# cjpatton/janus

Measured on AMD Instinct MI355X. Metric: helper reports/sec (prep_init+aggregate), Prio3SumVec len=1000 @1/2/4/8 GPU, higher is better.
Workload: dtype u32 (Field128 mod-p integer arithmetic, Keccak-p[1600,12]); 1 GPU; Prio3SumVec bits=8 length=1000 chunk_length=88: helper prep_init + prep_shares_to_prep + prep_next + aggregate; reports_per_gpu=1250000, parallelism=report-sharded x1 (RCCL all-gather + device mod-p combine)

## Files before the change

### janus_amd/csrc/jx_engine.cpp

```cpp
#include <hip/hip_runtime.h>

#include <cstdio>
#include <cstdlib>
#include <cstring>
#include <map>
#include <mutex>
#include <set>
#include <string>
#include <unordered_map>
#include <unordered_set>
#include <vector>

#include "jx_engine_internal.h"
#include "jx_field.h"
#include "jx_fused_plan.h"
#include "jx_sha_aes.h"
#include "jx_upload.h"

using namespace jx;
using namespace jxi;

static thread_local std::string t_err;

namespace jxi {
// ... 175 lines not shown
  c.P = next_pow2(1 + c.calls);
  if (mp && c.P > (1u << 30)) {
    why = "too many gadget calls for Field64";
    return JX_E_UNSUPPORTED;
  }
  c.logP = ilog2(c.P);
  c.gpoly_len = 2 * (c.P - 1) + 1;
  c.proof_len = arity + c.gpoly_len;
  c.ver_len = arity + 2;
  if (fp) {
    c.proof1_off = c.proof_len;
    c.proof_len += c.chunk1 + c.gpoly1_len;
    c.ver_len += c.chunk1 + 1;
  }
  const uint32_t fb = (c.algo == ALGO_COUNT || mp) ? 8 : 16;
  c.fb = fb;
  const bool jr = c.jr_len > 0;
  const uint32_t S = c.seed;
  c.ps_bytes = jr ? 2 * S : 0;
  c.his_bytes = jr ? 3 * S : 2 * S;
  c.lps_bytes = c.np * c.ver_len * fb + (jr ? S : 0);
  c.lis_bytes = (c.meas_len + c.np * c.proof_len) * fb + (jr ? S : 0);
  if (mp) {
    c.nco = MCOEF_K + 2 * c.calls;
    c.ncoef = 0;
    host_hmac_pads(vk, c.vk_ist, c.vk_ost);
    const uint8_t zero[32] = {0};
    host_hmac_pads(zero, c.zero_ist, c.zero_ost);
  } else if (c.algo == ALGO_COUNT)
    c.ncoef = 0;
  else if (c.algo == ALGO_SUM)
    c.ncoef = COEF_K + c.calls;
  else
    c.ncoef = COEF_K + 2 * c.calls;
  if (c.algo == ALGO_SUMVEC || c.algo == ALGO_HISTOGRAM || fp) {
    c.c_rpow = c.ncoef;
    c.ncoef += c.chunk;
    c.c_tpow = c.ncoef;
    c.ncoef += c.ngroups;
  }
  if (fp) {
    c.coef1 = c.ncoef;
    c.ncoef += G1_K + c.calls1;
  }
  for (int i = 0; i < 4; i++)
    c.vk[i] = (uint32_t)vk[4 * i] | ((uint32_t)vk[4 * i + 1] << 8) | ((uint32_t)vk[4 * i + 2] << 16) |
              ((uint32_t)vk[4 * i + 3] << 24);
  c.c_omega = 0;
  c.c_S = c.P;
  c.c_misc = c.P + c.gpoly_len;
  c.c_omega1 = c.c_misc + NMISC;
  c.c_S1 = c.c_omega1 + c.P1;
  return JX_OK;
}

static uint4 h_u4_64(uint64_t v) {
  uint4 r;
  r.x = lo32(v);
  r.y = hi32(v);
  r.z = r.w = 0;
  return r;
}

static void root_tables(f128 gen, uint32_t P, uint32_t logP, uint32_t calls, uint32_t glen, uint4* omega, uint4* S) {
  f128 w = gen;
  for (int i = 0; i < 66 - (int)logP; i++) w = mont128(w, w);
  f128 wk = make128(R1_128_LO, R1_128_HI);
// ... 2079 lines not shown
```

### janus_amd/csrc/jx_field.h

```cpp
#pragma once
#include <stdint.h>

#if defined(__HIPCC__) || defined(__HIP__)
#include <hip/hip_runtime.h>
#define JX_HD __host__ __device__ __forceinline__
#else
#define JX_HD static inline
#endif

namespace jx {


struct f128 {
  uint64_t lo, hi;
};

#if defined(__HIP_DEVICE_COMPILE__)
JX_HD uint32_t xor3(uint32_t a, uint32_t b, uint32_t c) { return __builtin_amdgcn_bitop3_b32(a, b, c, 0x96); }
JX_HD uint32_t maj3(uint32_t a, uint32_t b, uint32_t c) { return __builtin_amdgcn_bitop3_b32(a, b, c, 0xE8); }
#else
JX_HD uint32_t xor3(uint32_t a, uint32_t b, uint32_t c) { return a ^ b ^ c; }
JX_HD uint32_t maj3(uint32_t a, uint32_t b, uint32_t c) { return (a & b) ^ (a & c) ^ (b & c); }
#endif
JX_HD uint32_t lo32(uint64_t v) { return (uint32_t)v; }
// ... 271 lines not shown
  uint32_t c = 0;
  uint64_t a1 = addc64(w1, w2 * 28u, c);
  uint32_t b1 = b;
  a1 = subb64(a1, 0, b1);
  const uint64_t k = (uint64_t)(c - b1);
  uint32_t b2 = 0;
  a0 = subb64(a0, k, b2);
  a1 = a1 + 28u * k - b2;
  f128 v = make128(a0, a1);
  uint32_t br = 0;
  const uint64_t lo = subb64(v.lo, P128_LO, br);
  const uint64_t hi = subb64(v.hi, P128_HI, br);
  return ge_p128(v) ? make128(lo, hi) : v;
}
JX_HD void acc_add128(acc192& a, f128 v) { acc_add(a, v.lo, v.hi, 0); }
JX_HD f128 acc_reduce(const acc192& a) { return reduce192(a.w0, a.w1, a.w2); }


struct limbs26 {
  uint32_t l[5];
};
JX_HD limbs26 to_limbs26(f128 a) {
  const uint32_t M = (1u << 26) - 1;
  const uint32_t w0 = lo32(a.lo), w1 = hi32(a.lo), w2 = lo32(a.hi), w3 = hi32(a.hi);
  limbs26 r;
  r.l[0] = w0 & M;
  r.l[1] = (uint32_t)(((((uint64_t)w1) << 32) | w0) >> 26) & M;
  r.l[2] = (uint32_t)(((((uint64_t)w2) << 32) | w1) >> 20) & M;
  r.l[3] = (uint32_t)(((((uint64_t)w3) << 32) | w2) >> 14) & M;
  r.l[4] = w3 >> 8;
  return r;
}

struct wacc26 {
  uint64_t col[9];
};
JX_HD void wacc_zero(wacc26& a) {
#pragma unroll
  for (int s = 0; s < 9; s++) a.col[s] = 0;
}
JX_HD void wacc_mac(wacc26& a, const limbs26& x, const limbs26& c) {
#pragma unroll
  for (int i = 0; i < 5; i++)
#pragma unroll
    for (int j = 0; j < 5; j++) {
      a.col[i + j] += (uint64_t)x.l[i] * c.l[j];
#ifdef __HIP_DEVICE_COMPILE__
      asm("" : "+v"(a.col[i + j]));
#endif
    }
}
JX_HD void wacc_normalize(wacc26& a) {
  const uint64_t M = (1ull << 26) - 1;
#pragma unroll
  for (int s = 0; s < 8; s++) {
    a.col[s + 1] += a.col[s] >> 26;
    a.col[s] &= M;
  }
}
JX_HD f128 wacc_reduce(wacc26 a) {
  wacc_normalize(a);
  uint64_t o[5] = {0, 0, 0, 0, 0};
  int oi = 0, nb = 0;
  uint64_t buf_lo = 0, buf_hi = 0;
#pragma unroll
  for (int s = 0; s < 9; s++) {
// ... 165 lines not shown
```

### janus_amd/csrc/jx_flp.hip

```cpp
#include "jx_field.h"
#include "jx_kernels.h"

namespace jx {


__device__ __forceinline__ f128 ld_lead(const Bufs& b, const Cfg& c, uint64_t r, uint32_t idx, bool& dfail) {
  uint4 v = *reinterpret_cast<const uint4*>(b.lps + (uint64_t)c.lps_bytes * r + 16u * idx);
  f128 x = u4_to_f(v);
  dfail |= ge_p128(x);
  return x;
}

template <bool LEADER>
__global__ __launch_bounds__(256) void flp_sum_kernel(Cfg c, Bufs b) {
  const uint32_t lane = threadIdx.x & 63;
  const uint64_t blk = (uint64_t)blockIdx.x * 4 + (threadIdx.x >> 6);
  const uint64_t nblk = (b.n + 63) / 64;
  if (blk >= nblk) return;
  const uint64_t r0 = blk * 64 + lane;
  const uint64_t r = r0 < b.n ? r0 : b.n - 1;
  const uint32_t NC = c.ncoef, C = c.calls;
  const uint4* omega = b.consts + c.c_omega;
  f128 LR = ld_il(b.coef, blk, NC, COEF_L, lane), c0R = ld_il(b.coef, blk, NC, COEF_C0, lane);
  f128 tR = ld_il(b.coef, blk, NC, COEF_T, lane), rR = ld_il(b.coef, blk, NC, COEF_R, lane);
  acc192 ao;
  acc_zero(ao);
  const MeasView mv = meas_view(c, b, blk, lane);
  for (uint32_t k = 1; k <= C; k++) {
    f128 x = u4_to_f(mv[k - 1]);
    uint64_t lo, hi;
    uint32_t top;
    mont128_lazy(x, ld_il(b.coef, blk, NC, COEF_K + k - 1, lane), lo, hi, top);
// ... 44 lines not shown
    }
    return;
  }
  bool dfail = false;
  f128 lv = ld_lead(b, c, r, 0, dfail), lw = ld_lead(b, c, r, 1, dfail), lg = ld_lead(b, c, r, 2, dfail);
  const uint32_t flags = b.flags[r];
  uint32_t verdict = 0;
  if (flags & FLAG_INIT_FAIL)
    verdict = 1;
  else if (dfail)
    verdict = 2;
  else {
    f128 V0 = add128(v, lv), V1 = add128(W0, lw), VG = add128(G, lg);
    f128 lhs = sub128(mont128(V1, V1), mont128(V1, make128(1, 0)));
    if (!is_zero128(V0) || !eq128(lhs, mont128(VG, make128(1, 0))))
      verdict = 3;
    else if (flags & FLAG_NEXT_FAIL)
      verdict = 4;
  }
  if (r0 < b.n) b.verdicts[r0] = (uint8_t)verdict;
}

template <int PPW, bool HIST, bool LEADER>
__device__ __forceinline__ void psum_group_finish(const Cfg& c, const Bufs& b, uint64_t blk, uint32_t g, uint32_t lane,
                                                  const f128* E, const f128* O, f128 sxr);
template <int PPW, bool HIST, bool LEADER>
__device__ __forceinline__ void psum_part_finish(const Cfg& c, const Bufs& b, uint64_t blk, uint32_t g, uint32_t lane,
                                                 uint32_t kf, wacc26* ae, wacc26* ao, acc192& sx) {
  const uint32_t NG = c.ngroups;
  const uint64_t r0 = blk * 64 + lane;
  const uint64_t r = r0 < b.n ? r0 : b.n - 1;
  const uint32_t NC = c.ncoef, C = c.calls, chunk = c.chunk, M = c.meas_len, A = 2 * chunk;
  const uint32_t j0 = g * PPW;
  const uint4* coefb = b.coef + il_idx(blk, NC, 0, lane);
  const MeasView measb = meas_view(c, b, blk, lane);
#pragma unroll 1
  for (uint32_t k = kf + 1; k <= C; k++) {
    const limbs26 ck = to_limbs26(u4_to_f(coefb[(COEF_K + 2 * (k - 1)) * IL]));
    const limbs26 dk = to_limbs26(u4_to_f(coefb[(COEF_K + 2 * (k - 1) + 1) * IL]));
    const uint32_t nb = (k - 1) * chunk + j0;
#pragma unroll
    for (int i = 0; i < PPW; i++) {
      if (j0 + i < chunk && nb + i < M) {
        const f128 x = u4_to_f(measb[nb + i]);
        const limbs26 xl = to_limbs26(x);
        wacc_mac(ae[i], xl, dk);
        wacc_mac(ao[i], xl, ck);
        if (HIST) acc_add128(sx, x);
      }
    }
    if (((k - kf) & 511u) == 0) {
#pragma unroll
      for (int i = 0; i < PPW; i++) {
        wacc_normalize(ae[i]);
        wacc_normalize(ao[i]);
      }
    }
  }
  f128 E[PPW], O[PPW];
#pragma unroll
  for (int i = 0; i < PPW; i++) {
    E[i] = wacc_reduce(ae[i]);
    O[i] = wacc_reduce(ao[i]);
  }
  psum_group_finish<PPW, HIST, LEADER>(c, b, blk, g, lane, E, O, HIST ? acc_reduce(sx) : make128(0, 0));
}

template <int PPW, bool HIST, bool LEADER>
__device__ __forceinline__ void psum_group_finish(const Cfg& c, const Bufs& b, uint64_t blk, uint32_t g, uint32_t lane,
                                                  const f128* E, const f128* O, f128 sxr) {
  const uint32_t NG = c.ngroups;
  const uint64_t r0 = blk * 64 + lane;
// ... 40 lines not shown
      gpart = add128(mont128(gpart, tR), gm);
    }
    gpart = mont128(gpart, u4_to_f(coefb[(c.c_tpow + g) * IL]));
  }
  uint4* pp = b.part + ((blk * c.ngt + g) * 4) * IL + lane;
  pp[0] = f_to_u4(prod);
  pp[IL] = f_to_u4(vpart);
  pp[2 * IL] = f_to_u4(gpart);
  if (HIST) pp[3 * IL] = f_to_u4(sxr);
  if (dfail && r0 < b.n) atomicOr(&b.flags[r0], FLAG_DFAIL);
}

template <int PPW, bool HIST, bool LEADER, int PF = 1>
__global__ __launch_bounds__(64, 4) void flp_psum_part_kernel(Cfg c, Bufs b) {
  const uint32_t NG = c.ngroups;
  const uint32_t bid = blockIdx.x;
  const uint32_t xcd = bid & 7u, q = bid >> 3;
  const uint32_t g = q % NG;
  const uint64_t blk = (uint64_t)(q / NG) * 8 + xcd;
  const uint64_t nblk = (b.n + 63) / 64;
  if (blk >= nblk) return;
  const uint32_t lane = threadIdx.x;
  const uint32_t NC = c.ncoef, C = c.calls, chunk = c.chunk, M = c.meas_len;
  const uint32_t j0 = g * PPW;

  wacc26 ae[PPW], ao[PPW];
  acc192 sx;
#pragma unroll
  for (int i = 0; i < PPW; i++) {
    wacc_zero(ae[i]);
    wacc_zero(ao[i]);
  }
  acc_zero(sx);
  const uint4* coefb = b.coef + il_idx(blk, NC, 0, lane);
  const MeasView measb = meas_view(c, b, blk, lane);
  uint32_t kf = 0;
  if (j0 + PPW <= chunk && M >= j0 + PPW) kf = min(C, (M - j0 - PPW) / chunk + 1);
  for (uint32_t k0 = 1; k0 <= kf; k0 += 512) {
    const uint32_t k1 = min(kf, k0 + 511);
    uint4 cr[PF], dr[PF], xr[PF][PPW];
#pragma unroll
    for (int u = 0; u < PF; u++) {
      const uint32_t k = k0 + u;
      if (k <= k1) {
        cr[u] = coefb[(COEF_K + 2 * (k - 1)) * IL];
        dr[u] = coefb[(COEF_K + 2 * (k - 1) + 1) * IL];
#pragma unroll
        for (int i = 0; i < PPW; i++) xr[u][i] = measb[(uint64_t)((k - 1) * chunk + j0 + i)];
      }
    }
#pragma unroll 1
    for (uint32_t kb = k0; kb <= k1; kb += PF) {
#pragma unroll
      for (int u = 0; u < PF; u++) {
        const uint32_t k = kb + u;
        if (k <= k1) {
          const limbs26 ck = to_limbs26(u4_to_f(cr[u]));
          const limbs26 dk = to_limbs26(u4_to_f(dr[u]));
          f128 x[PPW];
#pragma unroll
          for (int i = 0; i < PPW; i++) x[i] = u4_to_f(xr[u][i]);
          const uint32_t kn = k + PF;
          if (kn <= k1) {
            cr[u] = coefb[(COEF_K + 2 * (kn - 1)) * IL];
            dr[u] = coefb[(COEF_K + 2 * (kn - 1) + 1) * IL];
#pragma unroll
            for (int i = 0; i < PPW; i++) xr[u][i] = measb[(uint64_t)((kn - 1) * chunk + j0 + i)];
          }
#pragma unroll
          for (int i = 0; i < PPW; i++) {
            const limbs26 xl = to_limbs26(x[i]);
            wacc_mac(ae[i], xl, dk);
            wacc_mac(ao[i], xl, ck);
            if (HIST) acc_add128(sx, x[i]);
          }
        }
      }
    }
#pragma unroll
    for (int i = 0; i < PPW; i++) {
      wacc_normalize(ae[i]);
      wacc_normalize(ao[i]);
    }
  }
  psum_part_finish<PPW, HIST, LEADER>(c, b, blk, g, lane, kf, ae, ao, sx);
}

template <int N>
__device__ __forceinline__ void wait_vmcnt() {
  static_assert(N >= 0 && N < 64, "vmcnt is 6 bits");
  __builtin_amdgcn_s_waitcnt(0x3f70 | (N & 15) | ((N >> 4) << 14));
}
__device__ __forceinline__ void glds16(const uint4* src, uint4* lds_row) {
  __builtin_amdgcn_global_load_lds((const void*)src, (void*)lds_row, 16, 0, 0);
}

constexpr uint32_t K3W = 4;
__device__ __forceinline__ uint32_t lds_addr(const void* p) {
  return (uint32_t)(size_t)(const __attribute__((address_space(3))) uint8_t*)p;
}
__device__ __forceinline__ void lds_read4(uint32_t a0, uint32_t a1, uint32_t a2, uint32_t a3, uint4& v0, uint4& v1,
                                          uint4& v2, uint4& v3) {
  asm volatile(
      "ds_read_b128 %0, %4\n\t"
      "ds_read_b128 %1, %5\n\t"
      "ds_read_b128 %2, %6\n\t"
      "ds_read_b128 %3, %7\n\t"
      "s_waitcnt lgkmcnt(0)"
      : "=&v"(v0), "=&v"(v1), "=&v"(v2), "=&v"(v3)
      : "v"(a0), "v"(a1), "v"(a2), "v"(a3)
      : "memory");
}
template <int PPW, bool HIST, bool LEADER, int D, int W = K3W, bool RING_ONLY = false>
__global__ __launch_bounds__(64 * W, 4) void flp_psum_part_glds_kernel(Cfg c, Bufs b) {
  static_assert(PPW == 2, "lds_read4 reads c, d and two measurement rows");
  constexpr int ROWS = 2 + W * PPW;
  __shared__ uint4 ring[D][ROWS][64];
  const uint32_t NG = c.ngroups, NW = (NG + W - 1) / W;
  const uint32_t bid = blockIdx.x, xcd = bid & 7u, q = bid >> 3;
  const uint32_t wg = q % NW;
  const uint64_t blk = (uint64_t)(q / NW) * 8 + xcd;
  const uint64_t nblk = (b.n + 63) / 64;
  if (blk >= nblk) return;
  const uint32_t wave = threadIdx.x >> 6, lane = threadIdx.x & 63;
  const uint32_t g = wg * W + wave;
  const uint32_t C = c.calls, chunk = c.chunk, M = c.meas_len;
  const uint32_t j0 = g * PPW;
  const uint4* coefb = b.coef + il_idx(blk, c.ncoef, 0, lane);
  const MeasView measb = meas_view(c, b, blk, lane);
  const uint4* zero = b.consts + c.c_misc + MISC_ZERO;
  const uint32_t kfw = C;
  bool real[PPW];
#pragma unroll
  for (int i = 0; i < PPW; i++) real[i] = g < NG && j0 + i < chunk;

  wacc26 ae[PPW], ao[PPW];
  acc192 sx;
#pragma unroll
  for (int i = 0; i < PPW; i++) {
    wacc_zero(ae[i]);
    wacc_zero(ao[i]);
  }
  acc_zero(sx);
  const bool inpl = LEADER && !HIST && b.meas_rs != 0;
  auto issue = [&](uint32_t k) {
    const uint32_t sl = (k - 1) % D;
    if (wave < 2) glds16(coefb + (uint64_t)(COEF_K + 2 * (k - 1) + wave) * IL, &ring[sl][wave][0]);
    if (inpl) {
      static_assert(W * PPW == 8, "one 128-byte row segment per report per call");
#pragma unroll
      for (int u = 0; u < PPW; u++) {
        const uint32_t q = wave * PPW + u, a = lane & 7u, p = (lane >> 3) ^ (q & 1u);
        const uint32_t slot = wg * (W * PPW) + p, e = (k - 1) * chunk + slot;
        const uint64_t r0 = blk * 64 + 8 * q + a, r = r0 < b.n ? r0 : b.n - 1;
        const uint4* src = slot < chunk && e < M ? reinterpret_cast<const uint4*>(b.meas_src + r * b.meas_rs) + e : zero;
        glds16(src, &ring[sl][2 + q][0]);
      }
    } else {
#pragma unroll
      for (int i = 0; i < PPW; i++) {
        const uint32_t e = (k - 1) * chunk + j0 + i;
        glds16(real[i] && e < M ? &measb[e] : zero, &ring[sl][2 + wave * PPW + i][0]);
      }
    }
  };
  auto wait_call = [&](bool tail) {
    if (tail) {
      wait_vmcnt<0>();
    } else if (wave < 2) {
      wait_vmcnt<(D - 2) * (PPW + 1)>();
    } else {
      wait_vmcnt<(D - 2) * PPW>();
    }
  };
  for (uint32_t k = 1; k < D && k <= kfw; k++) issue(k);
  const uint32_t ring_base = lds_addr(&ring[0][0][lane]);
  constexpr uint32_t SLOT_BYTES = ROWS * 64 * 16, ROW_BYTES = 64 * 16;
  uint32_t xoff[PPW];
#pragma unroll
  for (int i = 0; i < PPW; i++) {
    const uint32_t q = lane >> 3, p = wave * PPW + i;
    xoff[i] = inpl ? (2 + q) * ROW_BYTES + ((8 * (p ^ (q & 1u)) + (lane & 7u)) * 16) - lane * 16
                   : (2 + wave * PPW + i) * ROW_BYTES;
  }
#pragma unroll 1
  for (uint32_t k = 1; k <= kfw; k++) {
    wait_call(k + D - 2 > kfw);
    __builtin_amdgcn_s_barrier();
    if (k + D - 1 <= kfw) issue(k + D - 1);
    if (g < NG) {
      const uint32_t a = ring_base + ((k - 1) % D) * SLOT_BYTES;
      uint4 cv, dv, xv[PPW];
      lds_read4(a, a + ROW_BYTES, a + xoff[0], a + xoff[1], cv, dv, xv[0], xv[1]);
      const limbs26 ck = to_limbs26(u4_to_f(cv));
      const limbs26 dk = to_limbs26(u4_to_f(dv));
#pragma unroll
      for (int i = 0; i < PPW; i++) {
        const f128 x = u4_to_f(xv[i]);
        const limbs26 xl = to_limbs26(x);
        wacc_mac(ae[i], xl, dk);
        wacc_mac(ao[i], xl, ck);
        if (HIST) acc_add128(sx, x);
      }
      if ((k & 511u) == 0) {
#pragma unroll
        for (int i = 0; i < PPW; i++) {
          wacc_normalize(ae[i]);
          wacc_normalize(ao[i]);
        }
      }
    }
  }
  if (g >= NG) return;
  if constexpr (RING_ONLY) {
    uint64_t h = 0;
#pragma unroll
    for (int i = 0; i < PPW; i++)
#pragma unroll
      for (int q = 0; q < 9; q++) h ^= ae[i].col[q] ^ ao[i].col[q];
    b.part[((blk * c.ngt + g) * 4) * IL + lane] = make_uint4((uint32_t)h, (uint32_t)(h >> 32), 0, 0);
    return;
  }
  psum_part_finish<PPW, HIST, LEADER>(c, b, blk, g, lane, C, ae, ao, sx);
}

template <bool HIST, bool LEADER>
__global__ __launch_bounds__(256) void flp_psum_final_kernel(Cfg c, Bufs b) {
  const uint64_t r = (uint64_t)blockIdx.x * blockDim.x + threadIdx.x;
  if (r >= b.n) return;
  const uint64_t blk = r / 64;
  const uint32_t lane = r % 64, NG = c.ngroups, A = 2 * c.chunk;
  f128 P = make128(0, 0), V = make128(0, 0), G = make128(0, 0), SX = make128(0, 0);
  const uint4* pp = b.part + (blk * c.ngt * 4) * IL + lane;
  for (uint32_t g = 0; g < NG; g++, pp += 4 * IL) {
    P = add128(P, u4_to_f(pp[0]));
    V = add128(V, u4_to_f(pp[IL]));
    G = add128(G, u4_to_f(pp[2 * IL]));
    if (HIST) SX = add128(SX, u4_to_f(pp[3 * IL]));
  }
  f128 vh = V;
  if (HIST) {
    const f128 r2R = ld_il(b.coef, blk, c.ncoef, COEF_R2, lane);
    const f128 half = u4_to_f(b.consts[c.c_misc + 1]);
// ... 266 lines not shown
```

### janus_amd/csrc/jx_kernels.h

```cpp
#pragma once
#include <hip/hip_runtime.h>
#include <stdint.h>

#include "jx_flags.h"
#include "jx_k1_plan.h"
#include "jx_keyreg.h"

namespace jx {

enum Algo : uint32_t {
  ALGO_COUNT = 0,
  ALGO_SUM = 1,
  ALGO_SUMVEC = 2,
  ALGO_HISTOGRAM = 3,
  ALGO_SUMVEC_F64_MULTIPROOF = 4,
  ALGO_FIXEDPOINT_L2 = 5,
};
constexpr uint32_t MP_MAX_PROOFS = 8;

constexpr int IL = 64;

struct Cfg {
  uint32_t algo, bits, length, chunk;
  uint32_t meas_len, out_len, jr_len, proof_len, ver_len, calls, P, logP, gpoly_len;
  uint32_t ps_bytes, his_bytes, lps_bytes;
  uint32_t lis_bytes;
  uint32_t ncoef;
  uint32_t out_is_meas;
  uint32_t ppw, ngroups;
  uint32_t ngt;
  uint32_t vk[4];
  uint32_t c_omega, c_S, c_misc;
  uint32_t fb;
  uint32_t seed;
  uint32_t np;
  uint32_t dst_id;
  uint32_t nco;
  uint32_t vk_ist[8], vk_ost[8], zero_ist[8], zero_ost[8];
  uint32_t trunc_len;
  uint32_t qr_len;
  uint32_t norm_bits;
  uint32_t chunk1, calls1, P1, logP1, gpoly1_len, ppw1, ngroups1;
  uint32_t proof1_off;
  uint32_t coef1;
  uint32_t c_omega1, c_S1;
  uint32_t c_rpow, c_tpow;
};

enum : uint32_t {
  COEF_L = 0,
  COEF_C0 = 1,
  COEF_HALFSUM = 2,
  COEF_T = 3,
  COEF_R = 4,
  COEF_R2 = 5,
  COEF_K = 6,
};
enum : uint32_t {
  G1_L = 0,
  G1_C0 = 1,
  G1_T = 2,
  G1_K = 3,
};
constexpr uint32_t NMISC = 9;
constexpr uint32_t MISC_ZERO = 8;

struct Bufs {
  uint64_t n;
  const uint8_t* nonces;
  const uint8_t* ps;
  const uint8_t* his;
  const uint8_t* lps;
  const uint8_t* lis;
  uint64_t lis_rs;
  const uint8_t* vkeys;
  uint8_t* lps_out;
  uint32_t leader;
  uint4* meas;
  const uint8_t* meas_src;
  uint64_t meas_rs;
  uint4* proof;
  uint4* outs;
  uint4* coef;
  uint32_t* flags;
  uint4* part;
  uint8_t* verdicts;
  uint8_t* msgs;
  const uint4* consts;
  uint32_t force_slow;
};
// ... 106 lines not shown
  const uint8_t* cts;
  uint8_t* pts;
  const HpkeKeyRow* keys;
  uint32_t nkeys;
  const uint8_t* nonces;
  const uint8_t* ps;
  uint32_t ps_bytes;
  uint8_t* his;
  uint32_t his_bytes;
  uint8_t* status;
};

uint64_t k1_round_reports(const Cfg& c, int device);
Bufs bufs_tail(const Cfg& c, const Bufs& b, uint64_t S);
uint64_t mp_k1_round_reports(int device);
hipError_t launch_mp_xof(const Cfg& c, const Bufs& b, hipStream_t s);
hipError_t launch_mp_slow(const Cfg& c, const Bufs& b, hipStream_t s);
hipError_t launch_mp_flp(const Cfg& c, const Bufs& b, hipStream_t s);

inline uint32_t nblk_of(uint64_t n) { return (uint32_t)((n + 63) / 64); }

}

#if defined(__HIPCC__) || defined(__HIP__)
#include "jx_field.h"

namespace jx {

__device__ __forceinline__ uint64_t il_idx(uint64_t blk, uint32_t len, uint32_t e, uint32_t lane) {
  return (blk * len + e) * IL + lane;
}
#ifdef __HIP_DEVICE_COMPILE__
typedef __attribute__((address_space(1))) uint4 g_uint4;
#else
typedef uint4 g_uint4;
#endif
__device__ __forceinline__ f128 ld_il(const uint4* base, uint64_t blk, uint32_t len, uint32_t e, uint32_t lane) {
  return u4_to_f(((const g_uint4*)base)[il_idx(blk, len, e, lane)]);
}
__device__ __forceinline__ void st_il(uint4* base, uint64_t blk, uint32_t len, uint32_t e, uint32_t lane, f128 v) {
  ((g_uint4*)base)[il_idx(blk, len, e, lane)] = f_to_u4(v);
}
struct MeasView {
  const uint4* p;
  uint32_t es;
  __device__ __forceinline__ const uint4& operator[](uint64_t e) const { return p[e * es]; }
};
__device__ __forceinline__ MeasView meas_view(const Cfg& c, const Bufs& b, uint64_t blk, uint32_t lane) {
  if (b.meas_rs) {
    const uint64_t r0 = blk * 64 + lane, r = r0 < b.n ? r0 : b.n - 1;
    return MeasView{reinterpret_cast<const uint4*>(b.meas_src + r * b.meas_rs), 1u};
  }
  return MeasView{b.meas + il_idx(blk, c.meas_len, 0, lane), (uint32_t)IL};
}
__device__ __forceinline__ void load16(const uint8_t* p, uint32_t w[4]) {
  uint4 v = *reinterpret_cast<const uint4*>(p);
  w[0] = v.x;
  w[1] = v.y;
  w[2] = v.z;
  w[3] = v.w;
}

__device__ __forceinline__ void load_vk(const Cfg& c, const Bufs& b, uint64_t r, uint32_t vk[4]) {
  if (b.vkeys) {
    load16(b.vkeys + 16 * r, vk);
  } else {
#pragma unroll
    for (int i = 0; i < 4; i++) vk[i] = c.vk[i];
  }
}

__device__ __forceinline__ void trunc_add(acc192& a, f128 x, uint32_t sh) {
  uint64_t w0 = x.lo << sh;
  uint64_t w1 = sh ? ((x.hi << sh) | (x.lo >> (64 - sh))) : x.hi;
// ... 10 lines not shown
```

### janus_amd/csrc/jx_kernels.hip

```cpp
#include <cstdlib>
#include <stdlib.h>

#include <type_traits>

#include "jx_field.h"
#include "jx_kernels.h"
#include "jx_keccak.h"
#include "jx_sample.h"
#include "jx_sha256.h"

namespace jx {


__device__ uint64_t pow64(uint64_t a, uint64_t e) {
  uint64_t r = 1;
  while (e) {
    if (e & 1) r = mul64(r, a);
    a = mul64(a, a);
    e >>= 1;
  }
  return r;
}


// ... 136 lines not shown
template <bool WIDE, bool STORE = true>
__device__ __forceinline__ void emit_meas(const Cfg& c, uint4* mp, uint4* op, uint32_t e, uint4 v, uint32_t& gmax,
                                          TruncW& tr, f128& lo) {
  const bool in = e < c.meas_len;
  if (STORE && in) mp[(uint64_t)e * IL] = v;
  gmax = max(gmax, in ? ge_screen(v) : 0u);
  const bool tin = !c.out_is_meas && e < c.trunc_len;
  const uint32_t sh = opaque_u32(tin ? 1u << (WIDE ? (tr.j & 31u) : tr.j) : 0u);
  tr.T[0] += (uint64_t)v.x * sh;
  tr.T[1] += (uint64_t)v.y * sh;
  tr.T[2] += (uint64_t)v.z * sh;
  tr.T[3] += (uint64_t)v.w * sh;
  tr.j += tin ? 1u : 0u;
  if (WIDE && tin && tr.j == 32 && c.bits > 32) {
    lo = truncw_value(tr);
    truncw_zero(tr);
  }
  if (tin && tr.j == c.bits) {
    f128 val = truncw_value(tr);
    if (WIDE && c.bits > 32) val = add128(lo, shl32_mod(val));
    op[(uint64_t)tr.i * IL] = f_to_u4(val);
    truncw_zero(tr);
    tr.j = 0;
    tr.i++;
  }
}
__device__ __forceinline__ void emit_proof(const Cfg& c, uint4* pp, uint32_t e, uint4 v, uint32_t& gmax) {
  if (e >= c.proof_len) return;
  gmax = max(gmax, ge_screen(v));
  pp[(uint64_t)e * IL] = v;
}

__device__ f128 bary_coeffs(uint4* coef, uint64_t blk, uint32_t NC, uint32_t lane, f128 tR, const uint4* omega,
                            uint32_t C, uint32_t s0, uint32_t sk, uint32_t stride, bool with_d = false,
                            f128 rcR = f128{0, 0}) {
  auto slot = [&](uint32_t k) { return k == 0 ? s0 : sk + stride * (k - 1); };
  const g_uint4* gom = (const g_uint4*)omega;
  f128 acc = sub128(tR, u4_to_f(gom[0]));
  st_il(coef, blk, NC, slot(0), lane, acc);
  for (uint32_t k = 1; k <= C; k++) {
    acc = mont128(acc, sub128(tR, u4_to_f(gom[k])));
    st_il(coef, blk, NC, slot(k), lane, acc);
  }
  f128 inv, rp = make128(R1_128_LO, R1_128_HI), rinv = rp;
  if (with_d) {
    const f128 ie = minv(mont128(acc, rcR));
    inv = mont128(ie, rcR);
    rinv = mont128(ie, acc);
    rp = mpow(rcR, C - 1);
  } else {
    inv = minv(acc);
  }
  f128 sumc = make128(0, 0);
  auto pref = [&](int k) { return k >= 1 ? ld_il(coef, blk, NC, slot((uint32_t)k - 1), lane) : make128(0, 0); };
  auto wk = [&](int k) { return k >= 1 ? u4_to_f(gom[k]) : make128(0, 0); };
  const int Ci = (int)C;
  f128 q0 = pref(Ci), q1 = pref(Ci - 1), q2 = pref(Ci - 2), q3 = pref(Ci - 3);
  f128 o0 = wk(Ci), o1 = wk(Ci - 1), o2 = wk(Ci - 2), o3 = wk(Ci - 3);
  for (uint32_t k = C; k >= 1; k--) {
    const f128 pre = q0, w = o0;
    q0 = q1;
    q1 = q2;
    q2 = q3;
    o0 = o1;
    o1 = o2;
    o2 = o3;
    const uint32_t kn = k > 4 ? k - 4 : 1;
    q3 = ld_il(coef, blk, NC, slot(kn - 1), lane);
    o3 = u4_to_f(gom[kn]);
    f128 invden = mont128(inv, pre);
    inv = mont128(inv, sub128(tR, w));
    f128 ck = mont128(w, invden);
    st_il(coef, blk, NC, slot(k), lane, ck);
    if (with_d) {
      st_il(coef, blk, NC, slot(k) + 1, lane, mont128(ck, rp));
      rp = mont128(rp, rinv);
    }
    sumc = add128(sumc, ck);
  }
  st_il(coef, blk, NC, s0, lane, inv);
  return sumc;
}

template <bool INL = false>
__device__ uint32_t xof_tail(const Cfg& c, const Bufs& b, uint64_t blk, uint32_t lane, uint64_t r, bool write_msg,
                             const uint32_t nonce[4], const uint32_t part_l[4], const uint32_t lead_part[4],
                             const uint32_t part_h[4], uint32_t flags, bool slow) {
  uint32_t S[50];
  const uint32_t zero[4] = {0, 0, 0, 0};
  uint32_t corr[4];
  {
    Block m;
    blk_zero(m);
    int pos = blk_xof_prefix(m, c.dst_id, 6, zero);
#pragma unroll
    for (int i = 0; i < 4; i++) blk_put_word(m, pos + 4 * i, part_l[i]);
#pragma unroll
    for (int i = 0; i < 4; i++) blk_put_word(m, pos + 16 + 4 * i, part_h[i]);
    blk_pad(m, pos + 32);
    sponge_oneblock(S, m);
#pragma unroll
    for (int i = 0; i < 4; i++) corr[i] = S[i];
  }
  f128 jr[2];
  {
    Block m;
    blk_zero(m);
    int pos = blk_xof_prefix(m, c.dst_id, 3, corr);
    blk_put_byte(m, pos, 1);
// ... 20 lines not shown
  }
  if (write_msg) *reinterpret_cast<uint4*>(b.msgs + 16 * r) = make_uint4(msg[0], msg[1], msg[2], msg[3]);
  f128 tq[2];
  {
    Block m;
    blk_zero(m);
    uint32_t vk[4];
    load_vk(c, b, r, vk);
    int pos = blk_xof_prefix(m, c.dst_id, 5, vk);
    blk_put_byte(m, pos, 1);
#pragma unroll
    for (int i = 0; i < 4; i++) blk_put_word(m, pos + 1 + 4 * i, nonce[i]);
    blk_pad(m, pos + 17);
    sponge_oneblock(S, m);
    sample2_f128(S, tq, c.qr_len, slow, flags);
  }
  const f128 t = tq[0];
  const uint4* omega = b.consts + c.c_omega;
  const uint4* misc = b.consts + c.c_misc;
  const f128 R1 = make128(R1_128_LO, R1_128_HI);
  f128 tR = to_mont128(t);
  f128 tp = tR;
  for (uint32_t i = 0; i < c.logP; i++) tp = mont128(tp, tp);
  if (eq128(tp, R1)) flags |= FLAG_INIT_FAIL;
  f128 LR = mont128(sub128(tp, R1), u4_to_f(misc[0]));
  uint4* coef = b.coef;
  const uint32_t NC = c.ncoef;
  st_il(coef, blk, NC, COEF_L, lane, LR);
  st_il(coef, blk, NC, COEF_T, lane, tR);
  f128 rR = to_mont128(jr[0]);
  st_il(coef, blk, NC, COEF_R, lane, rR);
  st_il(coef, blk, NC, COEF_R2, lane, to_mont128(jr[1]));
  const uint32_t C = c.calls;
  const uint32_t stride = c.algo == ALGO_SUM ? 1u : 2u;
  const f128 rcR = mpow(rR, c.chunk);
  f128 sumc;
  if constexpr (INL) {
    [[clang::always_inline]] sumc =
        bary_coeffs(coef, blk, NC, lane, tR, omega, C, COEF_C0, COEF_K, stride, c.algo != ALGO_SUM, rcR);
  } else {
    sumc = bary_coeffs(coef, blk, NC, lane, tR, omega, C, COEF_C0, COEF_K, stride, c.algo != ALGO_SUM, rcR);
  }
  if (c.algo == ALGO_SUM) {
    st_il(coef, blk, NC, COEF_HALFSUM, lane, mont128(sumc, u4_to_f(misc[1])));
  } else {
    const f128 c0R = ld_il(coef, blk, NC, COEF_C0, lane);
    st_il(coef, blk, NC, COEF_C0, lane, mont128(c0R, LR));
    st_il(coef, blk, NC, COEF_L, lane, mont128(LR, make128(1, 0)));
    st_il(coef, blk, NC, COEF_HALFSUM, lane, mont128(mont128(sumc, LR), u4_to_f(misc[1])));
  }
  if (c.algo != ALGO_SUM) {
    f128 rj = mont128(LR, jr[0]);
    for (uint32_t j = 0; j < c.chunk; j++) {
      st_il(coef, blk, NC, c.c_rpow + j, lane, rj);
      rj = mont128(rj, rR);
    }
    const uint32_t per = (c.gpoly_len + c.ngroups - 1) / c.ngroups;
    const f128 tstep = mpow(tR, per);
    f128 tg = R1;
    for (uint32_t g = 0; g < c.ngroups; g++) {
      st_il(coef, blk, NC, c.c_tpow + g, lane, tg);
      tg = mont128(tg, tstep);
    }
  }
  if (c.algo == ALGO_FIXEDPOINT_L2) {
    const f128 t1R = to_mont128(tq[1]);
    f128 tp1 = t1R;
    for (uint32_t i = 0; i < c.logP1; i++) tp1 = mont128(tp1, tp1);
    if (eq128(tp1, R1)) flags |= FLAG_INIT_FAIL;
    const uint32_t B = c.coef1;
    st_il(coef, blk, NC, B + G1_L, lane, mont128(sub128(tp1, R1), u4_to_f(misc[7])));
    st_il(coef, blk, NC, B + G1_T, lane, t1R);
    if constexpr (INL) {
      [[clang::always_inline]] (void)bary_coeffs(coef, blk, NC, lane, t1R, b.consts + c.c_omega1, c.calls1, B + G1_C0,
                                                  B + G1_K, 1);
    } else {
      (void)bary_coeffs(coef, blk, NC, lane, t1R, b.consts + c.c_omega1, c.calls1, B + G1_C0, B + G1_K, 1);
    }
  }
  return flags;
}

constexpr uint32_t K1_WAVES = 4;
template <bool WIDE = false, int PROBE = 0>
__global__ __launch_bounds__(64 * K1_WAVES, 1) void xof_kernel(Cfg c, Bufs b) {
  const uint32_t lane = threadIdx.x & 63;
  const uint64_t blk = (uint64_t)blockIdx.x * K1_WAVES + (threadIdx.x >> 6);
  const uint64_t nblk = (b.n + 63) / 64;
  if (blk >= nblk) return;
  const uint64_t r0 = blk * 64 + lane;
  const uint64_t r = r0 < b.n ? r0 : b.n - 1;

  const uint8_t* hs = b.his + (uint64_t)c.his_bytes * r;
  uint32_t flags = 0;
  const uint32_t MB = c.meas_len * 16;
  const uint32_t ML = 42 + MB;
  const uint32_t NM = (MB + 167) / 168;
  const uint32_t b_last = ML / 168;

  uint32_t S[50], J[50];
  {
    uint32_t kmeas[4];
    load16(hs, kmeas);
    Block m;
    blk_zero(m);
    int pos = blk_xof_prefix(m, c.dst_id, 1, kmeas);
    blk_put_byte(m, pos, 1);
    blk_pad(m, pos + 1);
    sponge_oneblock(S, m);
  }
// ... 1336 lines not shown
```

Before: 7.794 million reports/s.

## Store per-call coefficients as packed 26-bit limbs and restructure glds pipeline

Result: faster. 7.896 million reports/s, median of 6 (+1.3%).

```diff
diff --git a/janus_amd/csrc/jx_engine.cpp b/janus_amd/csrc/jx_engine.cpp
--- a/janus_amd/csrc/jx_engine.cpp
+++ b/janus_amd/csrc/jx_engine.cpp
@@ -231,7 +231,7 @@
   else if (c.algo == ALGO_SUM)
     c.ncoef = COEF_K + c.calls;
   else
-    c.ncoef = COEF_K + 2 * c.calls;
+    c.ncoef = COEF_K + coef_call_slots(c.calls);
   if (c.algo == ALGO_SUMVEC || c.algo == ALGO_HISTOGRAM || fp) {
     c.c_rpow = c.ncoef;
     c.ncoef += c.chunk;
diff --git a/janus_amd/csrc/jx_field.h b/janus_amd/csrc/jx_field.h
--- a/janus_amd/csrc/jx_field.h
+++ b/janus_amd/csrc/jx_field.h
@@ -327,6 +327,27 @@
   return r;
 }
 
+constexpr int CD26_WORDS = 10;
+JX_HD void pack_cd26(f128 c, f128 d, uint32_t w[CD26_WORDS]) {
+  const limbs26 cl = to_limbs26(c), dl = to_limbs26(d);
+#pragma unroll
+  for (int i = 0; i < 4; i++) {
+    w[i] = cl.l[i];
+    w[4 + i] = dl.l[i];
+  }
+  w[8] = cl.l[4];
+  w[9] = dl.l[4];
+}
+JX_HD void unpack_cd26(const uint32_t w[CD26_WORDS], limbs26& c, limbs26& d) {
+#pragma unroll
+  for (int i = 0; i < 4; i++) {
+    c.l[i] = w[i];
+    d.l[i] = w[4 + i];
+  }
+  c.l[4] = w[8];
+  d.l[4] = w[9];
+}
+
 struct wacc26 {
   uint64_t col[9];
 };
diff --git a/janus_amd/csrc/jx_flp.hip b/janus_amd/csrc/jx_flp.hip
--- a/janus_amd/csrc/jx_flp.hip
+++ b/janus_amd/csrc/jx_flp.hip
@@ -1,3 +1,5 @@
+#include <type_traits>
+
 #include "jx_field.h"
 #include "jx_kernels.h"
 
@@ -108,12 +110,12 @@
   const uint64_t r = r0 < b.n ? r0 : b.n - 1;
   const uint32_t NC = c.ncoef, C = c.calls, chunk = c.chunk, M = c.meas_len, A = 2 * chunk;
   const uint32_t j0 = g * PPW;
-  const uint4* coefb = b.coef + il_idx(blk, NC, 0, lane);
+  const uint4* cblk = b.coef + il_idx(blk, NC, 0, 0);
   const MeasView measb = meas_view(c, b, blk, lane);
 #pragma unroll 1
   for (uint32_t k = kf + 1; k <= C; k++) {
-    const limbs26 ck = to_limbs26(u4_to_f(coefb[(COEF_K + 2 * (k - 1)) * IL]));
-    const limbs26 dk = to_limbs26(u4_to_f(coefb[(COEF_K + 2 * (k - 1) + 1) * IL]));
+    limbs26 ck, dk;
+    coef_call_limbs(ld_coef_call(cblk, lane, k), ck, dk);
     const uint32_t nb = (k - 1) * chunk + j0;
 #pragma unroll
     for (int i = 0; i < PPW; i++) {
@@ -220,19 +222,19 @@
     wacc_zero(ao[i]);
   }
   acc_zero(sx);
-  const uint4* coefb = b.coef + il_idx(blk, NC, 0, lane);
+  const uint4* cblk = b.coef + il_idx(blk, NC, 0, 0);
   const MeasView measb = meas_view(c, b, blk, lane);
   uint32_t kf = 0;
   if (j0 + PPW <= chunk && M >= j0 + PPW) kf = min(C, (M - j0 - PPW) / chunk + 1);
   for (uint32_t k0 = 1; k0 <= kf; k0 += 512) {
     const uint32_t k1 = min(kf, k0 + 511);
-    uint4 cr[PF], dr[PF], xr[PF][PPW];
+    CoefCall cr[PF];
+    uint4 xr[PF][PPW];
 #pragma unroll
     for (int u = 0; u < PF; u++) {
       const uint32_t k = k0 + u;
       if (k <= k1) {
-        cr[u] = coefb[(COEF_K + 2 * (k - 1)) * IL];
-        dr[u] = coefb[(COEF_K + 2 * (k - 1) + 1) * IL];
+        cr[u] = ld_coef_call(cblk, lane, k);
 #pragma unroll
         for (int i = 0; i < PPW; i++) xr[u][i] = measb[(uint64_t)((k - 1) * chunk + j0 + i)];
       }
@@ -243,15 +245,14 @@
       for (int u = 0; u < PF; u++) {
         const uint32_t k = kb + u;
         if (k <= k1) {
-          const limbs26 ck = to_limbs26(u4_to_f(cr[u]));
-          const limbs26 dk = to_limbs26(u4_to_f(dr[u]));
+          limbs26 ck, dk;
+          coef_call_limbs(cr[u], ck, dk);
           f128 x[PPW];
 #pragma unroll
           for (int i = 0; i < PPW; i++) x[i] = u4_to_f(xr[u][i]);
           const uint32_t kn = k + PF;
           if (kn <= k1) {
-            cr[u] = coefb[(COEF_K + 2 * (kn - 1)) * IL];
-            dr[u] = coefb[(COEF_K + 2 * (kn - 1) + 1) * IL];
+            cr[u] = ld_coef_call(cblk, lane, kn);
 #pragma unroll
             for (int i = 0; i < PPW; i++) xr[u][i] = measb[(uint64_t)((kn - 1) * chunk + j0 + i)];
           }
@@ -283,41 +284,52 @@
   __builtin_amdgcn_global_load_lds((const void*)src, (void*)lds_row, 16, 0, 0);
 }
 
+__device__ __forceinline__ void glds4(const uint32_t* src, uint32_t* lds_row) {
+  __builtin_amdgcn_global_load_lds((const void*)src, (void*)lds_row, 4, 0, 0);
+}
+
 constexpr uint32_t K3W = 4;
 __device__ __forceinline__ uint32_t lds_addr(const void* p) {
   return (uint32_t)(size_t)(const __attribute__((address_space(3))) uint8_t*)p;
 }
-__device__ __forceinline__ void lds_read4(uint32_t a0, uint32_t a1, uint32_t a2, uint32_t a3, uint4& v0, uint4& v1,
-                                          uint4& v2, uint4& v3) {
+template <uint32_t OC, uint32_t OX>
+__device__ __forceinline__ void lds_read_call(uint32_t ca, uint32_t ce, uint32_t x0, uint32_t x1, CoefCall& cv,
+                                              uint4& xv0, uint4& xv1) {
+  static_assert(OC + COEF_ROWB_U4 * 16 < 65536 && OX < 65536, "ds offsets are 16 bits");
   asm volatile(
-      "ds_read_b128 %0, %4\n\t"
-      "ds_read_b128 %1, %5\n\t"
-      "ds_read_b128 %2, %6\n\t"
-      "ds_read_b128 %3, %7\n\t"
+      "ds_read_b128 %0, %5 offset:%9\n\t"
+      "ds_read_b128 %1, %5 offset:%10\n\t"
+      "ds_read_b64 %2, %6 offset:%9\n\t"
+      "ds_read_b128 %3, %7 offset:%11\n\t"
+      "ds_read_b128 %4, %8 offset:%11\n\t"
       "s_waitcnt lgkmcnt(0)"
-      : "=&v"(v0), "=&v"(v1), "=&v"(v2), "=&v"(v3)
-      : "v"(a0), "v"(a1), "v"(a2), "v"(a3)
+      : "=&v"(cv.a), "=&v"(cv.b), "=&v"(cv.e), "=&v"(xv0), "=&v"(xv1)
+      : "v"(ca), "v"(ce), "v"(x0), "v"(x1), "n"(OC), "n"(OC + COEF_ROWB_U4 * 16), "n"(OX)
       : "memory");
 }
 template <int PPW, bool HIST, bool LEADER, int D, int W = K3W, bool RING_ONLY = false>
 __global__ __launch_bounds__(64 * W, 4) void flp_psum_part_glds_kernel(Cfg c, Bufs b) {
-  static_assert(PPW == 2, "lds_read4 reads c, d and two measurement rows");
-  constexpr int ROWS = 2 + W * PPW;
-  __shared__ uint4 ring[D][ROWS][64];
+  static_assert(PPW == 2, "lds_read_call reads two measurement rows");
+  static_assert(W == 4, "one quarter of a call's coefficient limbs per wave");
+  static_assert(D == 4, "the unrolled blocks assume measurement depth 4, coefficient depth 3");
+  constexpr int XROWS = W * PPW;
+  constexpr int DC = D - 1;
+  constexpr uint32_t ROW_BYTES = 64 * 16, XSLOT = XROWS * ROW_BYTES, XBYTES = D * XSLOT;
+  constexpr uint32_t CSLOT = COEF_CALL_BYTES;
+  __shared__ uint4 ring[D * XROWS * 64 + DC * COEF_CALL_U4];
+  static_assert(sizeof(ring) <= 40 * 1024, "four workgroups per CU");
   const uint32_t NG = c.ngroups, NW = (NG + W - 1) / W;
   const uint32_t bid = blockIdx.x, xcd = bid & 7u, q = bid >> 3;
   const uint32_t wg = q % NW;
   const uint64_t blk = (uint64_t)(q / NW) * 8 + xcd;
   const uint64_t nblk = (b.n + 63) / 64;
   if (blk >= nblk) return;
-  const uint32_t wave = threadIdx.x >> 6, lane = threadIdx.x & 63;
+  const uint32_t wave = __builtin_amdgcn_readfirstlane(threadIdx.x >> 6), lane = threadIdx.x & 63;
   const uint32_t g = wg * W + wave;
   const uint32_t C = c.calls, chunk = c.chunk, M = c.meas_len;
   const uint32_t j0 = g * PPW;
-  const uint4* coefb = b.coef + il_idx(blk, c.ncoef, 0, lane);
   const MeasView measb = meas_view(c, b, blk, lane);
   const uint4* zero = b.consts + c.c_misc + MISC_ZERO;
-  const uint32_t kfw = C;
   bool real[PPW];
 #pragma unroll
   for (int i = 0; i < PPW; i++) real[i] = g < NG && j0 + i < chunk;
@@ -331,72 +343,151 @@
   }
   acc_zero(sx);
   const bool inpl = LEADER && !HIST && b.meas_rs != 0;
-  auto issue = [&](uint32_t k) {
-    const uint32_t sl = (k - 1) % D;
-    if (wave < 2) glds16(coefb + (uint64_t)(COEF_K + 2 * (k - 1) + wave) * IL, &ring[sl][wave][0]);
+  static_assert(W * PPW == 8, "one 128-byte row segment per report per call");
+  const uint8_t* xbase[PPW];
+  bool xreal[PPW], xlast[PPW];
+#pragma unroll
+  for (int u = 0; u < PPW; u++) {
+    uint32_t xslot;
     if (inpl) {
-      static_assert(W * PPW == 8, "one 128-byte row segment per report per call");
-#pragma unroll
-      for (int u = 0; u < PPW; u++) {
-        const uint32_t q = wave * PPW + u, a = lane & 7u, p = (lane >> 3) ^ (q & 1u);
-        const uint32_t slot = wg * (W * PPW) + p, e = (k - 1) * chunk + slot;
-        const uint64_t r0 = blk * 64 + 8 * q + a, r = r0 < b.n ? r0 : b.n - 1;
-        const uint4* src = slot < chunk && e < M ? reinterpret_cast<const uint4*>(b.meas_src + r * b.meas_rs) + e : zero;
-        glds16(src, &ring[sl][2 + q][0]);
-      }
+      const uint32_t q = wave * PPW + u, a = lane & 7u, p = (lane >> 3) ^ (q & 1u);
+      const uint64_t r0 = blk * 64 + 8 * q + a, r = r0 < b.n ? r0 : b.n - 1;
+      xslot = wg * (W * PPW) + p;
+      xreal[u] = xslot < chunk;
+      xbase[u] = b.meas_src + r * b.meas_rs + 16ull * xslot;
     } else {
-#pragma unroll
-      for (int i = 0; i < PPW; i++) {
-        const uint32_t e = (k - 1) * chunk + j0 + i;
-        glds16(real[i] && e < M ? &measb[e] : zero, &ring[sl][2 + wave * PPW + i][0]);
-      }
-    }
+      xslot = j0 + u;
+      xreal[u] = real[u];
+      xbase[u] = reinterpret_cast<const uint8_t*>(&measb[xslot]);
+    }
+    xlast[u] = xreal[u] && (C - 1) * chunk + xslot < M;
+  }
+  const uint64_t xstep = (uint64_t)chunk * measb.es * 16u;
+  const uint32_t cq = wave < 2 ? wave * ROW_BYTES : COEF_ROWC_U4 * 16 + (wave - 2) * 256;
+  const uint8_t* cbase = reinterpret_cast<const uint8_t*>(b.coef + il_idx(blk, c.ncoef, COEF_K, 0)) + cq +
+                         (wave < 2 ? lane * 16 : lane * 4);
+  uint8_t* const ringb = reinterpret_cast<uint8_t*>(ring);
+  auto issue_c = [&](const uint8_t* src, uint32_t sc) {
+    uint8_t* dst = ringb + XBYTES + sc * CSLOT + cq;
+    if (wave < 2)
+      glds16(reinterpret_cast<const uint4*>(src), reinterpret_cast<uint4*>(dst));
+    else
+      glds4(reinterpret_cast<const uint32_t*>(src), reinterpret_cast<uint32_t*>(dst));
   };
-  auto wait_call = [&](bool tail) {
-    if (tail) {
-      wait_vmcnt<0>();
-    } else if (wave < 2) {
-      wait_vmcnt<(D - 2) * (PPW + 1)>();
-    } else {
-      wait_vmcnt<(D - 2) * PPW>();
-    }
+  auto issue_x = [&](const uint8_t* const* src, uint32_t sx_) {
+#pragma unroll
+    for (int u = 0; u < PPW; u++)
+      glds16(reinterpret_cast<const uint4*>(src[u]),
+             reinterpret_cast<uint4*>(ringb + sx_ * XSLOT + (wave * PPW + u) * ROW_BYTES));
   };
-  for (uint32_t k = 1; k < D && k <= kfw; k++) issue(k);
-  const uint32_t ring_base = lds_addr(&ring[0][0][lane]);
-  constexpr uint32_t SLOT_BYTES = ROWS * 64 * 16, ROW_BYTES = 64 * 16;
-  uint32_t xoff[PPW];
+  const uint8_t* xp[PPW];
+  uint64_t xst[PPW];
+#pragma unroll
+  for (int u = 0; u < PPW; u++) {
+    xp[u] = xreal[u] ? xbase[u] : reinterpret_cast<const uint8_t*>(zero);
+    xst[u] = xreal[u] ? xstep : 0u;
+  }
+  const uint8_t* cp = cbase;
+  auto step_x = [&]() {
+#pragma unroll
+    for (int u = 0; u < PPW; u++) {
+      xp[u] += xst[u];
+      asm volatile("" : "+v"(xp[u]));
+    }
+  };
+  auto issue_c_k = [&](uint32_t k) {
+    issue_c(cp, (k - 1) % DC);
+    cp += CSLOT;
+  };
+  auto issue_x_k = [&](uint32_t k) {
+    const uint8_t* src[PPW];
+#pragma unroll
+    for (int u = 0; u < PPW; u++)
+      src[u] = k < C || xlast[u] ? xp[u] : reinterpret_cast<const uint8_t*>(zero);
+    issue_x(src, (k - 1) % D);
+    step_x();
+  };
+  for (uint32_t k = 1; k < D && k <= C; k++) {
+    issue_x_k(k);
+    if (k < DC) issue_c_k(k);
+  }
+  const uint32_t ring_base = lds_addr(ring) + lane * 16;
+  uint32_t xa[PPW];
 #pragma unroll
   for (int i = 0; i < PPW; i++) {
     const uint32_t q = lane >> 3, p = wave * PPW + i;
-    xoff[i] = inpl ? (2 + q) * ROW_BYTES + ((8 * (p ^ (q & 1u)) + (lane & 7u)) * 16) - lane * 16
-                   : (2 + wave * PPW + i) * ROW_BYTES;
-  }
+    xa[i] = ring_base + (inpl ? q * ROW_BYTES + ((8 * (p ^ (q & 1u)) + (lane & 7u)) * 16) - lane * 16
+                              : (wave * PPW + i) * ROW_BYTES);
+  }
+  const uint32_t ca = ring_base, ce = lds_addr(ring) + COEF_ROWC_U4 * 16 + lane * 8;
+  auto mac_call = [&](const CoefCall& cv, const uint4* xv) {
+    limbs26 ck, dk;
+    coef_call_limbs(cv, ck, dk);
+#pragma unroll
+    for (int i = 0; i < PPW; i++) {
+      const f128 x = u4_to_f(xv[i]);
+      const limbs26 xl = to_limbs26(x);
+      wacc_mac(ae[i], xl, dk);
+      wacc_mac(ao[i], xl, ck);
+      if (HIST) acc_add128(sx, x);
+    }
+  };
+  auto normalize = [&]() {
+#pragma unroll
+    for (int i = 0; i < PPW; i++) {
+      wacc_normalize(ae[i]);
+      wacc_normalize(ao[i]);
+    }
+  };
+  uint32_t k = 1;
+  {
+    auto step = [&](auto uc, auto phc) {
+      constexpr uint32_t U = decltype(uc)::value, PH = decltype(phc)::value;
+      wait_vmcnt<2 * PPW + 1>();
+      __builtin_amdgcn_s_barrier();
+      issue_c(cp, (PH + U + DC - 1) % DC);
+      issue_x(xp, (U + D - 1) % D);
+      cp += CSLOT;
+      step_x();
+      if (g < NG) {
+        CoefCall cv;
+        uint4 xv[PPW];
+        lds_read_call<XBYTES + ((PH + U) % DC) * CSLOT, U * XSLOT>(ca, ce, xa[0], xa[1], cv, xv[0], xv[1]);
+        mac_call(cv, xv);
+      }
+    };
+    auto block = [&](auto phc) {
+      step(std::integral_constant<uint32_t, 0>{}, phc);
+      step(std::integral_constant<uint32_t, 1>{}, phc);
+      step(std::integral_constant<uint32_t, 2>{}, phc);
+      step(std::integral_constant<uint32_t, 3>{}, phc);
+      k += D;
+      if (((k - 1) & 511u) == 0 && g < NG) normalize();
+    };
+    const uint32_t nblocks = C > 2 * D - 1 ? (C - (2 * D - 1) + D - 1) / D : 0;
 #pragma unroll 1
-  for (uint32_t k = 1; k <= kfw; k++) {
-    wait_call(k + D - 2 > kfw);
+    for (uint32_t t = nblocks / DC; t > 0; t--) {
+      block(std::integral_constant<uint32_t, 0>{});
+      block(std::integral_constant<uint32_t, 1>{});
+      block(std::integral_constant<uint32_t, 2>{});
+    }
+  }
+#pragma unroll 1
+  for (; k <= C; k++) {
+    if (k + 2 > C)
+      wait_vmcnt<0>();
+    else
+      wait_vmcnt<2 * PPW + 1>();
     __builtin_amdgcn_s_barrier();
-    if (k + D - 1 <= kfw) issue(k + D - 1);
+    if (k + DC - 1 <= C) issue_c_k(k + DC - 1);
+    if (k + D - 1 <= C) issue_x_k(k + D - 1);
     if (g < NG) {
-      const uint32_t a = ring_base + ((k - 1) % D) * SLOT_BYTES;
-      uint4 cv, dv, xv[PPW];
-      lds_read4(a, a + ROW_BYTES, a + xoff[0], a + xoff[1], cv, dv, xv[0], xv[1]);
-      const limbs26 ck = to_limbs26(u4_to_f(cv));
-      const limbs26 dk = to_limbs26(u4_to_f(dv));
-#pragma unroll
-      for (int i = 0; i < PPW; i++) {
-        const f128 x = u4_to_f(xv[i]);
-        const limbs26 xl = to_limbs26(x);
-        wacc_mac(ae[i], xl, dk);
-        wacc_mac(ao[i], xl, ck);
-        if (HIST) acc_add128(sx, x);
-      }
-      if ((k & 511u) == 0) {
-#pragma unroll
-        for (int i = 0; i < PPW; i++) {
-          wacc_normalize(ae[i]);
-          wacc_normalize(ao[i]);
-        }
-      }
+      const uint32_t co = ((k - 1) % DC) * CSLOT, xo = ((k - 1) % D) * XSLOT;
+      CoefCall cv;
+      uint4 xv[PPW];
+      lds_read_call<XBYTES, 0>(ca + co, ce + co, xa[0] + xo, xa[1] + xo, cv, xv[0], xv[1]);
+      mac_call(cv, xv);
+      if ((k & 511u) == 0) normalize();
     }
   }
   if (g >= NG) return;
diff --git a/janus_amd/csrc/jx_kernels.h b/janus_amd/csrc/jx_kernels.h
--- a/janus_amd/csrc/jx_kernels.h
+++ b/janus_amd/csrc/jx_kernels.h
@@ -56,6 +56,10 @@
   COEF_R2 = 5,
   COEF_K = 6,
 };
+constexpr uint32_t COEF_CALL_U4 = 2 * IL + IL / 2;
+constexpr uint32_t COEF_ROWB_U4 = IL, COEF_ROWC_U4 = 2 * IL;
+constexpr uint32_t COEF_CALL_BYTES = COEF_CALL_U4 * 16;
+inline uint32_t coef_call_slots(uint32_t calls) { return (5 * calls + 1) / 2; }
 enum : uint32_t {
   G1_L = 0,
   G1_C0 = 1,
@@ -228,14 +232,40 @@
 }
 #ifdef __HIP_DEVICE_COMPILE__
 typedef __attribute__((address_space(1))) uint4 g_uint4;
+typedef __attribute__((address_space(1))) uint2 g_uint2;
 #else
 typedef uint4 g_uint4;
+typedef uint2 g_uint2;
 #endif
 __device__ __forceinline__ f128 ld_il(const uint4* base, uint64_t blk, uint32_t len, uint32_t e, uint32_t lane) {
   return u4_to_f(((const g_uint4*)base)[il_idx(blk, len, e, lane)]);
 }
 __device__ __forceinline__ void st_il(uint4* base, uint64_t blk, uint32_t len, uint32_t e, uint32_t lane, f128 v) {
   ((g_uint4*)base)[il_idx(blk, len, e, lane)] = f_to_u4(v);
+}
+struct CoefCall {
+  uint4 a, b;
+  uint2 e;
+};
+__device__ __forceinline__ CoefCall ld_coef_call(const uint4* cblk, uint32_t lane, uint32_t k) {
+  const g_uint4* p = (const g_uint4*)cblk + (uint64_t)COEF_K * IL + (uint64_t)(k - 1) * COEF_CALL_U4;
+  CoefCall v;
+  v.a = p[lane];
+  v.b = p[COEF_ROWB_U4 + lane];
+  v.e = ((const g_uint2*)(p + COEF_ROWC_U4))[lane];
+  return v;
+}
+__device__ __forceinline__ void coef_call_limbs(const CoefCall& v, limbs26& c, limbs26& d) {
+  const uint32_t w[CD26_WORDS] = {v.a.x, v.a.y, v.a.z, v.a.w, v.b.x, v.b.y, v.b.z, v.b.w, v.e.x, v.e.y};
+  unpack_cd26(w, c, d);
+}
+__device__ __forceinline__ void st_coef_call(uint4* cblk, uint32_t lane, uint32_t k, f128 c, f128 d) {
+  uint32_t w[CD26_WORDS];
+  pack_cd26(c, d, w);
+  g_uint4* p = (g_uint4*)cblk + (uint64_t)COEF_K * IL + (uint64_t)(k - 1) * COEF_CALL_U4;
+  p[lane] = make_uint4(w[0], w[1], w[2], w[3]);
+  p[COEF_ROWB_U4 + lane] = make_uint4(w[4], w[5], w[6], w[7]);
+  ((g_uint2*)(p + COEF_ROWC_U4))[lane] = make_uint2(w[8], w[9]);
 }
 struct MeasView {
   const uint4* p;
diff --git a/janus_amd/csrc/jx_kernels.hip b/janus_amd/csrc/jx_kernels.hip
--- a/janus_amd/csrc/jx_kernels.hip
+++ b/janus_amd/csrc/jx_kernels.hip
@@ -192,15 +192,18 @@
 }
 
 __device__ f128 bary_coeffs(uint4* coef, uint64_t blk, uint32_t NC, uint32_t lane, f128 tR, const uint4* omega,
-                            uint32_t C, uint32_t s0, uint32_t sk, uint32_t stride, bool with_d = false,
-                            f128 rcR = f128{0, 0}) {
-  auto slot = [&](uint32_t k) { return k == 0 ? s0 : sk + stride * (k - 1); };
+                            uint32_t C, uint32_t s0, uint32_t sk, bool with_d = false, f128 rcR = f128{0, 0}) {
+  auto slot = [&](uint32_t k) -> uint64_t {
+    if (k == 0) return il_idx(blk, NC, s0, lane);
+    return with_d ? il_idx(blk, NC, sk, lane) + (uint64_t)(k - 1) * COEF_CALL_U4 : il_idx(blk, NC, sk + (k - 1), lane);
+  };
+  g_uint4* gco = (g_uint4*)coef;
   const g_uint4* gom = (const g_uint4*)omega;
   f128 acc = sub128(tR, u4_to_f(gom[0]));
-  st_il(coef, blk, NC, slot(0), lane, acc);
+  gco[slot(0)] = f_to_u4(acc);
   for (uint32_t k = 1; k <= C; k++) {
     acc = mont128(acc, sub128(tR, u4_to_f(gom[k])));
-    st_il(coef, blk, NC, slot(k), lane, acc);
+    gco[slot(k)] = f_to_u4(acc);
   }
   f128 inv, rp = make128(R1_128_LO, R1_128_HI), rinv = rp;
   if (with_d) {
@@ -212,7 +215,7 @@
     inv = minv(acc);
   }
   f128 sumc = make128(0, 0);
-  auto pref = [&](int k) { return k >= 1 ? ld_il(coef, blk, NC, slot((uint32_t)k - 1), lane) : make128(0, 0); };
+  auto pref = [&](int k) { return k >= 1 ? u4_to_f(gco[slot((uint32_t)k - 1)]) : make128(0, 0); };
   auto wk = [&](int k) { return k >= 1 ? u4_to_f(gom[k]) : make128(0, 0); };
   const int Ci = (int)C;
   f128 q0 = pref(Ci), q1 = pref(Ci - 1), q2 = pref(Ci - 2), q3 = pref(Ci - 3);
@@ -226,15 +229,16 @@
     o1 = o2;
     o2 = o3;
     const uint32_t kn = k > 4 ? k - 4 : 1;
-    q3 = ld_il(coef, blk, NC, slot(kn - 1), lane);
+    q3 = u4_to_f(gco[slot(kn - 1)]);
     o3 = u4_to_f(gom[kn]);
     f128 invden = mont128(inv, pre);
     inv = mont128(inv, sub128(tR, w));
     f128 ck = mont128(w, invden);
-    st_il(coef, blk, NC, slot(k), lane, ck);
     if (with_d) {
-      st_il(coef, blk, NC, slot(k) + 1, lane, mont128(ck, rp));
+      st_coef_call(coef + il_idx(blk, NC, 0, 0), lane, k, ck, mont128(ck, rp));
       rp = mont128(rp, rinv);
+    } else {
+      gco[slot(k)] = f_to_u4(ck);
     }
     sumc = add128(sumc, ck);
   }
@@ -321,14 +325,13 @@
   st_il(coef, blk, NC, COEF_R, lane, rR);
   st_il(coef, blk, NC, COEF_R2, lane, to_mont128(jr[1]));
   const uint32_t C = c.calls;
-  const uint32_t stride = c.algo == ALGO_SUM ? 1u : 2u;
   const f128 rcR = mpow(rR, c.chunk);
   f128 sumc;
   if constexpr (INL) {
     [[clang::always_inline]] sumc =
-        bary_coeffs(coef, blk, NC, lane, tR, omega, C, COEF_C0, COEF_K, stride, c.algo != ALGO_SUM, rcR);
+        bary_coeffs(coef, blk, NC, lane, tR, omega, C, COEF_C0, COEF_K, c.algo != ALGO_SUM, rcR);
   } else {
-    sumc = bary_coeffs(coef, blk, NC, lane, tR, omega, C, COEF_C0, COEF_K, stride, c.algo != ALGO_SUM, rcR);
+    sumc = bary_coeffs(coef, blk, NC, lane, tR, omega, C, COEF_C0, COEF_K, c.algo != ALGO_SUM, rcR);
   }
   if (c.algo == ALGO_SUM) {
     st_il(coef, blk, NC, COEF_HALFSUM, lane, mont128(sumc, u4_to_f(misc[1])));
@@ -362,9 +365,9 @@
     st_il(coef, blk, NC, B + G1_T, lane, t1R);
     if constexpr (INL) {
       [[clang::always_inline]] (void)bary_coeffs(coef, blk, NC, lane, t1R, b.consts + c.c_omega1, c.calls1, B + G1_C0,
-                                                  B + G1_K, 1);
+                                                  B + G1_K);
     } else {
-      (void)bary_coeffs(coef, blk, NC, lane, t1R, b.consts + c.c_omega1, c.calls1, B + G1_C0, B + G1_K, 1);
+      (void)bary_coeffs(coef, blk, NC, lane, t1R, b.consts + c.c_omega1, c.calls1, B + G1_C0, B + G1_K);
     }
   }
   return flags;
```
